# facebookresearch/GPU-DPF

Hardware: NVIDIA B200
Metric: DPFs/sec (higher is better)
Workload: dtype u32

## Files before the change

### gpu-dpf_b200/csrc/dpf_core.cuh

```cuda
#pragma once

#include <stdint.h>

#if defined(__CUDACC__)
#define DPF_HD __host__ __device__ __forceinline__
#else
#define DPF_HD inline __attribute__((always_inline))
#endif

#if defined(__CUDA_ARCH__)
#define DPF_UNROLL _Pragma("unroll")
#else
#define DPF_UNROLL
#endif

#if defined(__CUDA_ARCH__)
#define DPF_DEVICE_CODE 1
#else
#define DPF_DEVICE_CODE 0
#endif

namespace b200dpf {

enum : int { PRF_DUMMY = 0, PRF_SALSA20 = 1, PRF_CHACHA20 = 2, PRF_AES128 = 3 };

struct Seed {
    uint32_t x, y, z, w;
};

DPF_HD Seed make_seed(uint32_t x, uint32_t y, uint32_t z, uint32_t w)
{
    Seed s; s.x = x; s.y = y; s.z = z; s.w = w; return s;
}


DPF_HD uint32_t rotl(uint32_t v, int r)
{
#if DPF_DEVICE_CODE
    return __funnelshift_l(v, v, r);
#else
    return (v << r) | (v >> (32 - r));
#endif
}

#ifndef DPF_FMA_ROT_MASK
#define DPF_FMA_ROT_MASK 0
#endif
template <int R>
DPF_HD uint32_t rotl_fma(uint32_t v)
{
#if DPF_DEVICE_CODE
    uint32_t lo, hi;
    asm("{\n\t.reg .u64 t;\n\tmul.wide.u32 t, %2, %3;\n\tmov.b64 {%0,%1}, t;\n\t}"
        : "=r"(lo), "=r"(hi) : "r"(v), "n"(1u << R));
    return lo + hi;
#else
    return (v << R) | (v >> (32 - R));
#endif
}
template <int SLOT, int R>
DPF_HD uint32_t rot_sel(uint32_t v)
{
    return ((DPF_FMA_ROT_MASK >> SLOT) & 1) ? rotl_fma<R>(v) : rotl(v, R);
}

DPF_HD uint32_t prmt(uint32_t a, uint32_t b, uint32_t sel)
{
#if DPF_DEVICE_CODE
    return __byte_perm(a, b, sel);
#else
    uint64_t ab = ((uint64_t)b << 32) | a;
    uint32_t r = 0;
    for (int i = 0; i < 4; i++) {
        uint32_t n = (sel >> (4 * i)) & 7u;
        r |= (uint32_t)((ab >> (8 * n)) & 0xffu) << (8 * i);
    }
    return r;
#endif
}

DPF_HD Seed add128(const Seed &a, const Seed &b)
{
    Seed r;
#if DPF_DEVICE_CODE
    asm("add.cc.u32 %0, %4, %8;\n\t"
        "addc.cc.u32 %1, %5, %9;\n\t"
        "addc.cc.u32 %2, %6, %10;\n\t"
        "addc.u32 %3, %7, %11;"
        : "=r"(r.x), "=r"(r.y), "=r"(r.z), "=r"(r.w)
        : "r"(a.x), "r"(a.y), "r"(a.z), "r"(a.w), "r"(b.x), "r"(b.y), "r"(b.z), "r"(b.w));
#else
    uint64_t c = (uint64_t)a.x + b.x;
    r.x = (uint32_t)c; c >>= 32;
    c += (uint64_t)a.y + b.y; r.y = (uint32_t)c; c >>= 32;
    c += (uint64_t)a.z + b.z; r.z = (uint32_t)c; c >>= 32;
    c += (uint64_t)a.w + b.w; r.w = (uint32_t)c;
#endif
    return r;
}

DPF_HD Seed dummy_prf(const Seed &s, uint32_t pos)
{
    const uint64_t k = 4242ull + pos;
    Seed r;
    uint64_t t = (uint64_t)s.x * k + k;
    r.x = (uint32_t)t; t >>= 32;
    t += (uint64_t)s.y * k; r.y = (uint32_t)t; t >>= 32;
    t += (uint64_t)s.z * k; r.z = (uint32_t)t; t >>= 32;
    t += (uint64_t)s.w * k; r.w = (uint32_t)t;
    return r;
}

#define DPF_SIGMA0 0x65787061u
#define DPF_SIGMA1 0x6e642033u
#define DPF_SIGMA2 0x322d6279u
#define DPF_SIGMA3 0x7465206bu

#define DPF_SALSA_QR(a, b, c, d)      \
    do {                              \
        b ^= rot_sel<0, 7>(a + d);    \
        c ^= rot_sel<1, 9>(b + a);    \
        d ^= rot_sel<2, 13>(c + b);   \
        a ^= rot_sel<3, 18>(d + c);   \
    } while (0)

#define DPF_CHACHA_QR(a, b, c, d)     \
    do {                              \
        a += b; d = rot_sel<0, 16>(d ^ a);  \
        c += d; b = rot_sel<1, 12>(b ^ c);  \
        a += b; d = rot_sel<2, 8>(d ^ a);   \
        c += d; b = rot_sel<3, 7>(b ^ c);   \
    } while (0)

template <bool LEAF>
DPF_HD Seed salsa12(const Seed &s, uint32_t pos)
{
    const uint32_t i1 = s.w, i2 = s.z, i3 = s.y, i4 = s.x;
    uint32_t x0 = DPF_SIGMA0, x1 = i1, x2 = i2, x3 = i3, x4 = i4, x5 = DPF_SIGMA1, x6 = 0, x7 = 0,
             x8 = 0, x9 = pos, x10 = DPF_SIGMA2, x11 = 0, x12 = 0, x13 = 0, x14 = 0, x15 = DPF_SIGMA3;
DPF_UNROLL
    for (int r = 0; r < 6; r++) {
        DPF_SALSA_QR(x0, x4, x8, x12);
        DPF_SALSA_QR(x5, x9, x13, x1);
        DPF_SALSA_QR(x10, x14, x2, x6);
        DPF_SALSA_QR(x15, x3, x7, x11);
        DPF_SALSA_QR(x0, x1, x2, x3);
        DPF_SALSA_QR(x5, x6, x7, x4);
        DPF_SALSA_QR(x10, x11, x8, x9);
        DPF_SALSA_QR(x15, x12, x13, x14);
    }
    Seed o;
    o.x = x4 + i4;
    if (LEAF) { o.y = 0; o.z = 0; o.w = 0; }
    else { o.y = x3 + i3; o.z = x2 + i2; o.w = x1 + i1; }
    return o;
}

template <bool LEAF>
DPF_HD Seed chacha12(const Seed &s, uint32_t pos)
{
    const uint32_t i4 = s.w, i5 = s.z, i6 = s.y, i7 = s.x;
    uint32_t x0 = DPF_SIGMA0, x1 = DPF_SIGMA1, x2 = DPF_SIGMA2, x3 = DPF_SIGMA3, x4 = i4, x5 = i5, x6 = i6,
             x7 = i7, x8 = 0, x9 = 0, x10 = 0, x11 = 0, x12 = 0, x13 = pos, x14 = 0, x15 = 0;
DPF_UNROLL
    for (int r = 0; r < 6; r++) {
        DPF_CHACHA_QR(x0, x4, x8, x12);
        DPF_CHACHA_QR(x1, x5, x9, x13);
        DPF_CHACHA_QR(x2, x6, x10, x14);
        DPF_CHACHA_QR(x3, x7, x11, x15);
        DPF_CHACHA_QR(x0, x5, x10, x15);
        DPF_CHACHA_QR(x1, x6, x11, x12);
        DPF_CHACHA_QR(x2, x7, x8, x13);
        DPF_CHACHA_QR(x3, x4, x9, x14);
    }
    Seed o;
    o.x = x7 + i7;
    if (LEAF) { o.y = 0; o.z = 0; o.w = 0; }
    else { o.y = x6 + i6; o.z = x5 + i5; o.w = x4 + i4; }
    return o;
}

struct AesHostTables {
    const uint32_t *te0;
    template <int K, int BYTE>
    DPF_HD uint32_t te(uint32_t word) const
    {
        uint32_t v = te0[(word >> (8 * BYTE)) & 0xffu];
        return K == 0 ? v : rotl(v, 8 * K);
    }
};

template <class TA, int B0, int B1, int B2, int B3>
DPF_HD uint32_t aes_sub4(const TA &ta, uint32_t w0, uint32_t w1, uint32_t w2, uint32_t w3)
{
    const uint32_t a = ta.template te<2, B0>(w0);
    const uint32_t b = ta.template te<3, B1>(w1);
    const uint32_t c = ta.template te<0, B2>(w2);
    const uint32_t d = ta.template te<1, B3>(w3);
    const uint32_t ab = prmt(a, b, 0x0050);
    const uint32_t cd = prmt(c, d, 0x7200);
    return prmt(ab, cd, 0x7610);
}

template <class TA>
DPF_HD void aes_next_rk(const TA &ta, uint32_t &k0, uint32_t &k1, uint32_t &k2, uint32_t &k3, uint32_t rc)
{
    const uint32_t t = aes_sub4<TA, 1, 2, 3, 0>(ta, k3, k3, k3, k3);
    k0 ^= t ^ rc;
    k1 ^= k0;
    k2 ^= k1;
    k3 ^= k2;
}

template <class TA>
DPF_HD void aes_round(const TA &ta, uint32_t &s0, uint32_t &s1, uint32_t &s2, uint32_t &s3,
                      uint32_t k0, uint32_t k1, uint32_t k2, uint32_t k3)
{
    const uint32_t t0 = ta.template te<0, 0>(s0) ^ ta.template te<1, 1>(s1) ^ ta.template te<2, 2>(s2) ^ ta.template te<3, 3>(s3) ^ k0;
    const uint32_t t1 = ta.template te<0, 0>(s1) ^ ta.template te<1, 1>(s2) ^ ta.template te<2, 2>(s3) ^ ta.template te<3, 3>(s0) ^ k1;
    const uint32_t t2 = ta.template te<0, 0>(s2) ^ ta.template te<1, 1>(s3) ^ ta.template te<2, 2>(s0) ^ ta.template te<3, 3>(s1) ^ k2;
    const uint32_t t3 = ta.template te<0, 0>(s3) ^ ta.template te<1, 1>(s0) ^ ta.template te<2, 2>(s1) ^ ta.template te<3, 3>(s2) ^ k3;
    s0 = t0; s1 = t1; s2 = t2; s3 = t3;
}

template <class TA>
DPF_HD void aes_first_round(const TA &ta, uint32_t pos, uint32_t &k0, uint32_t &k1, uint32_t &k2, uint32_t &k3,
                            uint32_t &a0, uint32_t &a1, uint32_t &a2, uint32_t &a3, uint32_t &col0_te0)
{
    const uint32_t s0 = k0 ^ pos;
    const uint32_t l00 = ta.template te<0, 0>(s0), l11 = ta.template te<1, 1>(k1), l22 = ta.template te<2, 2>(k2), l33 = ta.template te<3, 3>(k3);
    const uint32_t l01 = ta.template te<0, 0>(k1), l12 = ta.template te<1, 1>(k2), l23 = ta.template te<2, 2>(k3), l30 = ta.template te<3, 3>(s0);
    const uint32_t l02 = ta.template te<0, 0>(k2), l13 = ta.template te<1, 1>(k3), l20 = ta.template te<2, 2>(s0), l31 = ta.template te<3, 3>(k1);
    const uint32_t l03 = ta.template te<0, 0>(k3), l10 = ta.template te<1, 1>(s0), l21 = ta.template te<2, 2>(k1), l32 = ta.template te<3, 3>(k2);
    const uint32_t ab = prmt(l13, l23, 0x0042);
    const uint32_t cd = prmt(l33, l03, 0x5000);
    const uint32_t t = prmt(ab, cd, 0x7610);
    k0 ^= t ^ 1u;
    k1 ^= k0;
    k2 ^= k1;
    k3 ^= k2;
    a0 = l00 ^ l11 ^ l22 ^ l33 ^ k0;
    a1 = l01 ^ l12 ^ l23 ^ l30 ^ k1;
    a2 = l02 ^ l13 ^ l20 ^ l31 ^ k2;
    a3 = l03 ^ l10 ^ l21 ^ l32 ^ k3;
    col0_te0 = l00;
}

template <bool LEAF, class TA>
DPF_HD void aes128_pair(const TA &ta, const Seed &s, Seed &c0, Seed &c1)
{
    uint32_t k0 = s.x, k1 = s.y, k2 = s.z, k3 = s.w;
    uint32_t a0, a1, a2, a3, l00;
    const uint32_t sib = ta.template te<0, 0>(k0 ^ 1u);
    aes_first_round(ta, 0u, k0, k1, k2, k3, a0, a1, a2, a3, l00);
    uint32_t b0 = a0 ^ l00 ^ sib, b1 = a1, b2 = a2, b3 = a3;
    uint32_t rc = 2;
DPF_UNROLL
    for (int r = 2; r <= 9; r++) {
        aes_next_rk(ta, k0, k1, k2, k3, rc);
        rc = (rc << 1) ^ ((rc & 0x80u) ? 0x11bu : 0u);
        aes_round(ta, a0, a1, a2, a3, k0, k1, k2, k3);
        aes_round(ta, b0, b1, b2, b3, k0, k1, k2, k3);
    }
    aes_next_rk(ta, k0, k1, k2, k3, rc);
    c0.x = aes_sub4<TA, 0, 1, 2, 3>(ta, a0, a1, a2, a3) ^ k0;
    c1.x = aes_sub4<TA, 0, 1, 2, 3>(ta, b0, b1, b2, b3) ^ k0;
    if (LEAF) {
        c0.y = c0.z = c0.w = 0;
        c1.y = c1.z = c1.w = 0;
    } else {
        c0.y = aes_sub4<TA, 0, 1, 2, 3>(ta, a1, a2, a3, a0) ^ k1;
        c0.z = aes_sub4<TA, 0, 1, 2, 3>(ta, a2, a3, a0, a1) ^ k2;
        c0.w = aes_sub4<TA, 0, 1, 2, 3>(ta, a3, a0, a1, a2) ^ k3;
        c1.y = aes_sub4<TA, 0, 1, 2, 3>(ta, b1, b2, b3, b0) ^ k1;
        c1.z = aes_sub4<TA, 0, 1, 2, 3>(ta, b2, b3, b0, b1) ^ k2;
        c1.w = aes_sub4<TA, 0, 1, 2, 3>(ta, b3, b0, b1, b2) ^ k3;
    }
}

template <class TA>
DPF_HD Seed aes128_one(const TA &ta, const Seed &s, uint32_t pos)
{
    uint32_t k0 = s.x, k1 = s.y, k2 = s.z, k3 = s.w;
    uint32_t a0, a1, a2, a3, l00;
    aes_first_round(ta, pos, k0, k1, k2, k3, a0, a1, a2, a3, l00);
    uint32_t rc = 2;
DPF_UNROLL
    for (int r = 2; r <= 9; r++) {
        aes_next_rk(ta, k0, k1, k2, k3, rc);
        rc = (rc << 1) ^ ((rc & 0x80u) ? 0x11bu : 0u);
        aes_round(ta, a0, a1, a2, a3, k0, k1, k2, k3);
    }
    aes_next_rk(ta, k0, k1, k2, k3, rc);
    Seed c;
    c.x = aes_sub4<TA, 0, 1, 2, 3>(ta, a0, a1, a2, a3) ^ k0;
    c.y = aes_sub4<TA, 0, 1, 2, 3>(ta, a1, a2, a3, a0) ^ k1;
    c.z = aes_sub4<TA, 0, 1, 2, 3>(ta, a2, a3, a0, a1) ^ k2;
    c.w = aes_sub4<TA, 0, 1, 2, 3>(ta, a3, a0, a1, a2) ^ k3;
    return c;
}


template <int PRF, bool LEAF, class TA>
DPF_HD void expand_pair(const TA &ta, const Seed &parent, Seed &c0, Seed &c1)
{
    if (PRF == PRF_DUMMY) {
        c0 = dummy_prf(parent, 0);
        c1 = dummy_prf(parent, 1);
    } else if (PRF == PRF_SALSA20) {
        c0 = salsa12<LEAF>(parent, 0);
        c1 = salsa12<LEAF>(parent, 1);
    } else if (PRF == PRF_CHACHA20) {
        c0 = chacha12<LEAF>(parent, 0);
        c1 = chacha12<LEAF>(parent, 1);
    } else {
        aes128_pair<LEAF>(ta, parent, c0, c1);
    }
}

template <int PRF, class TA>
DPF_HD Seed expand_one(const TA &ta, const Seed &parent, uint32_t pos)
{
    if (PRF == PRF_DUMMY) return dummy_prf(parent, pos);
    if (PRF == PRF_SALSA20) return salsa12<false>(parent, pos);
    if (PRF == PRF_CHACHA20) return chacha12<false>(parent, pos);
    return aes128_one(ta, parent, pos);
}


template <int PRF, class Env>
DPF_HD Seed walk_down(Env &env, Seed seed, int first_level, int steps, uint32_t q)
{
    for (int k = 0; k < steps; k++) {
        const uint32_t bit = (q >> (steps - 1 - k)) & 1u;
        const int level = first_level - k;
        const uint32_t bank = seed.x & 1u;
        seed = add128(expand_one<PRF>(env.ta, seed, bit), env.cw(level, bank, bit));
    }
    return seed;
}

DPF_HD int ctz32(uint32_t v)
{
#if DPF_DEVICE_CODE
    return __ffs((int)v) - 1;
#else
    return __builtin_ctz(v);
#endif
}

template <int PRF, bool FULL, class Env>
DPF_HD void eval_subtree(Env &env, Seed seed, int s, int level_base)
{
    int h = s;
    const uint32_t npairs = 1u << (s - 1);
    for (uint32_t i = 0; i < npairs; i++) {
        while (h > 1) {
            Seed c0, c1;
            expand_pair<PRF, false>(env.ta, seed, c0, c1);
            const uint32_t bank = seed.x & 1u;
            const int level = level_base + h - 1;
            c1 = add128(c1, env.cw(level, bank, 1));
            env.push(h - 1, c1);
            seed = add128(c0, env.cw(level, bank, 0));
            h--;
        }
        Seed l0, l1;
        const uint32_t bank = seed.x & 1u;
        if (FULL) {
            expand_pair<PRF, false>(env.ta, seed, l0, l1);
            env.node_pair(2 * i, add128(l0, env.cw(level_base, bank, 0)), add128(l1, env.cw(level_base, bank, 1)));
        } else {
            env.leaf_prefetch(2 * i);
            expand_pair<PRF, true>(env.ta, seed, l0, l1);
            env.leaf_pair(2 * i, l0.x + env.cw_lo(bank, 0), l1.x + env.cw_lo(bank, 1));
        }
        h = ctz32(i + 1) + 1;
        if (h < s) seed = env.pop(h);
    }
}

}
```

### gpu-dpf_b200/csrc/dpf_kernels.cu

```cuda
#include "dpf_kernels.cuh"

#include <algorithm>
#include <atomic>

#include "dpf_core.cuh"

namespace b200dpf {

namespace {

__constant__ uint32_t c_te0[256];

struct AesSmemTables {
    uint32_t lanebase;

    template <int K, int BYTE>
    __device__ __forceinline__ uint32_t te(uint32_t word) const
    {
        const uint32_t addr = __byte_perm(word, lanebase, 0x7604u | (BYTE << 4));
        uint32_t v;
        asm("ld.shared.u32 %0, [%1+%2];" : "=r"(v) : "r"(addr), "n"((K & 1) * 128 + (K >> 1) * 65536));
        return v;
    }
};

struct NoTables {
    template <int K, int BYTE>
    __device__ __forceinline__ uint32_t te(uint32_t) const { return 0; }
};

template <int PRF> struct TablePolicy { typedef NoTables type; };
template <> struct TablePolicy<PRF_AES128> { typedef AesSmemTables type; };

namespace tma {

__device__ __forceinline__ void mbar_init(uint32_t bar, uint32_t count)
{
    asm volatile("mbarrier.init.shared::cta.b64 [%0], %1;" ::"r"(bar), "r"(count));
}
__device__ __forceinline__ void mbar_expect_tx(uint32_t bar, uint32_t bytes)
{
    asm volatile("mbarrier.arrive.expect_tx.shared::cta.b64 _, [%0], %1;" ::"r"(bar), "r"(bytes) : "memory");
}
__device__ __forceinline__ void mbar_arrive(uint32_t bar)
{
    asm volatile("mbarrier.arrive.shared::cta.b64 _, [%0];" ::"r"(bar) : "memory");
}
__device__ __forceinline__ void mbar_wait(uint32_t bar, uint32_t parity)
{
    uint32_t done = 0;
    for (uint32_t spin = 0; !done; spin++) {
        asm volatile("{\n\t.reg .pred p;\n\tmbarrier.try_wait.parity.shared::cta.b64 p, [%1], %2;\n\tselp.u32 %0, 1, 0, p;\n\t}"
                     : "=r"(done) : "r"(bar), "r"(parity) : "memory");
        if (spin > (1u << 28)) __trap();
    }
}
__device__ __forceinline__ void bulk_g2s(uint32_t dst, const void *src, uint32_t bytes, uint32_t bar)
{
    asm volatile("cp.async.bulk.shared::cluster.global.mbarrier::complete_tx::bytes [%0], [%1], %2, [%3];"
                 ::"r"(dst), "l"(src), "r"(bytes), "r"(bar) : "memory");
}

}

template <int PRF, int NV, int THREADS, int MODE>
struct DevEnv {
    typename TablePolicy<PRF>::type ta;
    const uint4 *cw_lane;
    const uint32_t *cwlo_lane;
    uint4 *stack_lo, *stack_hi;
    int stack_split;
    const uint4 *rows;
    uint32_t row_stride_v;
    uint32_t acc[4 * NV];
    uint4 ra[4], rb[4];
    uint32_t *leaf_out;
    uint4 *front_out;
    uint32_t kpw;
    uint32_t *share_row;
    uint32_t pos_base;
    int depth;
    bool key_valid;

    __device__ __forceinline__ Seed cw(int level, uint32_t bank, uint32_t bit) const
    {
        const uint4 v = cw_lane[((level * 2 + (int)bank) * 2 + (int)bit) * 32];
        return make_seed(v.x, v.y, v.z, v.w);
    }
    __device__ __forceinline__ uint32_t cw_lo(uint32_t bank, uint32_t bit) const
    {
        return cwlo_lane[(bank * 2 + bit) * 32];
    }
    __device__ __forceinline__ uint4 *slot(int h) const
    {
        const int l = h - 1;
        return (l < stack_split ? stack_lo : stack_hi) + l * THREADS;
    }
    __device__ __forceinline__ void push(int h, const Seed &s) const
    {
        *slot(h) = make_uint4(s.x, s.y, s.z, s.w);
    }
    __device__ __forceinline__ Seed pop(int h) const
    {
        const uint4 v = *slot(h);
        return make_seed(v.x, v.y, v.z, v.w);
    }
    static constexpr bool MAC = (MODE == MODE_FUSED || MODE == MODE_GROUPED || MODE == MODE_FUSED_TMA);
    static constexpr bool STAGED = (MODE == MODE_FUSED_TMA);
    const uint4 *tile;
    uint32_t tile_bar;
    uint32_t tile_phase;
    bool tile_pending;

    __device__ __forceinline__ void leaf_prefetch(uint32_t local_pos)
    {
        if (STAGED) {
            if (tile_pending) {
                tma::mbar_wait(tile_bar, tile_phase);
                tile_phase ^= 1u;
                tile_pending = false;
            }
            const uint4 *r = tile + (size_t)local_pos * 4;
#pragma unroll
            for (int j = 0; j < 4; j++) ra[j] = r[j];
#pragma unroll
            for (int j = 0; j < 4; j++) rb[j] = r[4 + j];
        } else if (MAC) {
            const uint4 *r = rows + (size_t)local_pos * row_stride_v;
#pragma unroll
            for (int j = 0; j < 4; j++) ra[j] = __ldg(r + j);
#pragma unroll
            for (int j = 0; j < 4; j++) rb[j] = __ldg(r + row_stride_v + j);
        }
    }
    __device__ __forceinline__ void leaf_pair(uint32_t local_pos, uint32_t v0, uint32_t v1)
    {
        if (MAC) {
            if (leaf_out != nullptr) {
                leaf_out[(size_t)local_pos * 32] = v0;
                leaf_out[(size_t)(local_pos + 1) * 32] = v1;
            }
            const uint4 *r = rows + (size_t)local_pos * row_stride_v;
#pragma unroll
            for (int c = 0; c < NV / 4; c++) {
                uint4 na[4], nb[4];
                if (c + 1 < NV / 4) {
#pragma unroll
                    for (int j = 0; j < 4; j++) na[j] = __ldg(r + 4 * (c + 1) + j);
#pragma unroll
                    for (int j = 0; j < 4; j++) nb[j] = __ldg(r + row_stride_v + 4 * (c + 1) + j);
                }
#pragma unroll
                for (int j = 0; j < 4; j++) {
                    acc[16 * c + 4 * j + 0] += v0 * ra[j].x + v1 * rb[j].x;
                    acc[16 * c + 4 * j + 1] += v0 * ra[j].y + v1 * rb[j].y;
                    acc[16 * c + 4 * j + 2] += v0 * ra[j].z + v1 * rb[j].z;
                    acc[16 * c + 4 * j + 3] += v0 * ra[j].w + v1 * rb[j].w;
                }
                if (c + 1 < NV / 4) {
#pragma unroll
                    for (int j = 0; j < 4; j++) { ra[j] = na[j]; rb[j] = nb[j]; }
                }
            }
        } else if (MODE == MODE_EXPAND && key_valid) {
            const uint32_t p = pos_base + local_pos;
            share_row[__brev(p) >> (32 - depth)] = v0;
            share_row[__brev(p + 1) >> (32 - depth)] = v1;
        }
    }
    __device__ __forceinline__ void node_pair(uint32_t local_pos, const Seed &c0, const Seed &c1)
    {
        front_out[(size_t)local_pos * kpw] = make_uint4(c0.x, c0.y, c0.z, c0.w);
        front_out[(size_t)(local_pos + 1) * kpw] = make_uint4(c1.x, c1.y, c1.z, c1.w);
    }
};

template <int PRF, int NV> struct KernelShape { enum { THREADS = (NV <= 8 ? 256 : 384), MIN_BLOCKS = (NV <= 8 ? 2 : 1) }; };
#ifndef DPF_AES_THREADS
#define DPF_AES_THREADS 384
#endif
template <int NV> struct KernelShape<PRF_AES128, NV> { enum { THREADS = (NV <= 8 ? DPF_AES_THREADS : 256), MIN_BLOCKS = 1 }; };

extern __shared__ __align__(16) unsigned char g_dyn_smem[];

__device__ __forceinline__ void grid_barrier(uint32_t *bar, uint32_t target)
{
    __syncthreads();
    if (threadIdx.x == 0) {
        __threadfence();
        atomicAdd(bar, 1u);
        for (uint32_t spin = 0;; spin++) {
            uint32_t v;
            asm volatile("ld.acquire.gpu.global.u32 %0, [%1];" : "=r"(v) : "l"(bar) : "memory");
            if ((int32_t)(v - target) >= 0) break;
            if (spin > (1u << 25)) __trap();
            __nanosleep(40);
        }
        __threadfence();
    }
    __syncthreads();
}

__device__ __forceinline__ unsigned long long global_ns()
{
    unsigned long long t;
    asm volatile("mov.u64 %0, %globaltimer;" : "=l"(t));
    return t;
}

template <int PRF, int NV, int THREADS, int MODE>
__device__ __forceinline__ void run_phase(const EvalParams &p, const PhaseParams &ph,
                                          const typename TablePolicy<PRF>::type &ta, uint32_t quota = 0xffffffffu)
{
    const int tid = threadIdx.x;
    const int lane = tid & 31;

    uint4 *cw_s = reinterpret_cast<uint4 *>(g_dyn_smem + p.off_cw);
    uint32_t *cwlo_s = reinterpret_cast<uint32_t *>(g_dyn_smem + p.off_cwlo);
    uint4 *root_s = reinterpret_cast<uint4 *>(g_dyn_smem + p.off_root);
    volatile int *flag_s = reinterpret_cast<volatile int *>(g_dyn_smem + p.off_flag);

    const int kpw = 1 << p.kpw_log2;
    const int spw_log2 = 5 - p.kpw_log2;
    const int kslot = lane & (kpw - 1);
    const uint32_t sslot = (uint32_t)lane >> p.kpw_log2;
    const uint32_t ntickets = ph.nsub >> spw_log2;

    DevEnv<PRF, NV, THREADS, MODE> env;
    env.ta = ta;
    env.cw_lane = cw_s + kslot;
    env.cwlo_lane = cwlo_s + kslot;
    env.kpw = (uint32_t)kpw;
    env.stack_lo = reinterpret_cast<uint4 *>(g_dyn_smem + p.off_stack_lo) + tid;
    env.stack_hi = reinterpret_cast<uint4 *>(g_dyn_smem + p.off_stack_hi) + tid - ph.stack_split * THREADS;
    env.stack_split = ph.stack_split;
    env.row_stride_v = p.row_stride_v;
    env.depth = p.depth;
    if constexpr (MODE == MODE_FUSED_TMA) {
        const int w = tid >> 5;
        env.tile = reinterpret_cast<const uint4 *>(g_dyn_smem + p.off_tile + ((size_t)w << (ph.s + 6)));
        env.tile_bar = (uint32_t)__cvta_generic_to_shared(g_dyn_smem + p.off_tile_bar + 8 * w);
        env.tile_phase = 0;
        env.tile_pending = false;
        if (lane == 0) {
            tma::mbar_init(env.tile_bar, 1);
            asm volatile("fence.mbarrier_init.release.cluster;" ::: "memory");
        }
        __syncwarp();
    }

    constexpr bool GROUPED = (MODE == MODE_GROUPED);
    uint32_t taken = 0;
    for (int j = 0; j < p.key_groups; j++) {
        const int kg = (int)((blockIdx.x + (unsigned)j) % (unsigned)p.key_groups);

        int g_depth = p.depth, g_s = ph.s, g_walk_first = ph.walk_first_level, g_walk_steps = ph.walk_steps;
        int g_key_first = kg * kpw, g_key_last = p.nkeys - 1;
        uint32_t g_tickets = ntickets;
        const uint4 *g_table = p.table;
        if (GROUPED) {
            const GroupDesc g = p.groups[kg];
            g_depth = g.depth;
            g_s = g.s;
            g_walk_first = g.depth - 1;
            g_walk_steps = g.depth - g.s;
            g_key_first = (int)g.key_first;
            g_key_last = (int)(g.key_first + g.nkeys) - 1;
            g_tickets = g.nsub;
            g_table = p.table + g.table_off_v;
        }

        if (quota != 0xffffffffu && __syncthreads_and(taken >= quota)) break;
        if (tid == 0) *flag_s = (*reinterpret_cast<volatile uint32_t *>(ph.counters + kg) < g_tickets) ? 1 : 0;
        __syncthreads();
        const bool has_work = (*flag_s != 0);
        if (has_work) {
            const int per_key = g_depth * 4;
            for (int i = tid; i < per_key * kpw; i += THREADS) {
                const int k = i / per_key;
                const int e = i - k * per_key;
                const int bank = e / (g_depth * 2);
                const int lb = e - bank * (g_depth * 2);
                int key = g_key_first + k;
                if (key > g_key_last) key = g_key_last;
                const int level = lb >> 1, bit = lb & 1;
                const uint32_t slot = p.key_compact ? 2u + 4u * (uint32_t)level + 2u * (uint32_t)bank + (uint32_t)bit
                                                    : (bank ? 65u : 1u) + (uint32_t)lb;
                const uint4 v = __ldg(p.keys + (size_t)key * p.key_stride_v + slot);
                cw_s[((level * 2 + bank) * 2 + bit) * 32 + k] = v;
                if (level == 0) cwlo_s[(bank * 2 + bit) * 32 + k] = v.x;
            }
            if (tid < kpw) {
                int key = g_key_first + tid;
                if (key > g_key_last) key = g_key_last;
                root_s[tid] = __ldg(p.keys + (size_t)key * p.key_stride_v + p.key_root_v);
            }
        }
        __syncthreads();
        if (!has_work) continue;

        const int key = g_key_first + kslot;
        env.key_valid = key <= g_key_last;
        if (MODE == MODE_FUSED || MODE == MODE_FUSED_TMA || GROUPED) {
#pragma unroll
            for (int e = 0; e < 4 * NV; e++) env.acc[e] = 0;
        } else if (MODE == MODE_EXPAND) {
            env.share_row = p.shares + (size_t)(env.key_valid ? key : 0) * p.n;
        }
        const uint4 rv = root_s[kslot];
        const Seed root = make_seed(rv.x, rv.y, rv.z, rv.w);

        const uint32_t grid_warps = gridDim.x * (uint32_t)(THREADS / 32);
        const bool chunked = quota == 0xffffffffu;
        const bool ahead = g_s <= 4;
        uint32_t chunk = 1;
        if (chunked) chunk = min(8u, max(1u, g_tickets / (8u * grid_warps)));
        uint32_t t_raw = 0;
        bool draw = taken < quota;
        if (draw && lane == 0) t_raw = atomicAdd(ph.counters + kg, chunk);
        while (draw) {
            const uint32_t t0 = __shfl_sync(0xffffffffu, t_raw, 0);
            if (t0 >= g_tickets) break;
            const uint32_t t1 = min(t0 + chunk, g_tickets);
            taken += t1 - t0;
            draw = taken < quota;
            if (chunked) chunk = min(8u, max(1u, (g_tickets - t1) / (8u * grid_warps)));
            if (ahead && draw && lane == 0) t_raw = atomicAdd(ph.counters + kg, chunk);
          for (uint32_t t = t0; t < t1; t++) {
            const uint32_t q = (t << spw_log2) + sslot;
            Seed start = root;
            if (ph.frontier_in != nullptr) {
                const uint4 fv = __ldcg(ph.frontier_in + ((size_t)kg * p.nfront + (q >> ph.front_shift)) * kpw + kslot);
                start = make_seed(fv.x, fv.y, fv.z, fv.w);
            }
            const Seed r = walk_down<PRF>(env, start, g_walk_first, g_walk_steps, ph.sub_first + q);
            if (MODE == MODE_FRONTIER) {
                env.front_out = p.frontier_out + ((size_t)kg * p.nfront + ((size_t)q << g_s)) * kpw + kslot;
                eval_subtree<PRF, true>(env, r, g_s, ph.level_base);
            } else {
                env.rows = g_table + ((size_t)q << g_s) * p.row_stride_v + p.col_off_v;
                if constexpr (MODE == MODE_FUSED_TMA) {
                    __syncwarp();
                    if (lane == 0) {
                        asm volatile("fence.proxy.async.shared::cta;" ::: "memory");
                        const uint32_t bytes = 64u << g_s;
                        tma::mbar_expect_tx(env.tile_bar, bytes);
                        tma::bulk_g2s((uint32_t)__cvta_generic_to_shared(const_cast<uint4 *>(env.tile)), env.rows, bytes, env.tile_bar);
                    }
                    env.tile_pending = true;
                }
                env.pos_base = (ph.sub_first + q) << g_s;
                env.leaf_out = (!GROUPED && p.leaf_cache) ? p.leaf_cache + ((size_t)kg * p.n_local + ((size_t)q << g_s)) * 32 + lane
                                                          : nullptr;
                eval_subtree<PRF, false>(env, r, g_s, 0);
            }
          }
            if (!ahead && draw && lane == 0) t_raw = atomicAdd(ph.counters + kg, chunk);
        }

        if (MODE == MODE_FUSED || MODE == MODE_FUSED_TMA || GROUPED) {
            for (int off = kpw; off < 32; off <<= 1) {
#pragma unroll
                for (int e = 0; e < 4 * NV; e++) env.acc[e] += __shfl_xor_sync(0xffffffffu, env.acc[e], off);
            }
            if (env.key_valid && sslot == 0) {
                uint32_t *o = p.out + (size_t)key * p.out_stride + p.col_off;
#pragma unroll
                for (int e = 0; e < 4 * NV; e++)
                    if ((uint32_t)e < p.ncols) atomicAdd(o + e, env.acc[e]);
            }
        }
        __syncthreads();
    }
}

template <int PRF, int NV, int MODE>
__global__ void __launch_bounds__((KernelShape<PRF, NV>::THREADS), (KernelShape<PRF, NV>::MIN_BLOCKS))
dpf_eval_kernel(const __grid_constant__ EvalParams p)
{
    constexpr int THREADS = KernelShape<PRF, NV>::THREADS;
    const int tid = threadIdx.x;
    unsigned long long *stamp = (p.timing != nullptr && tid == 0) ? p.timing + (size_t)blockIdx.x * 8 : nullptr;
    if (stamp) stamp[0] = global_ns();

    typename TablePolicy<PRF>::type ta;
    if constexpr (PRF == PRF_AES128) {
        const uint32_t tab = (uint32_t)__cvta_generic_to_shared(g_dyn_smem + p.off_tab);
        if ((tab & 0xffffu) != 0) __trap();
        for (int i = tid; i < 256 * 32; i += THREADS) {
            const uint32_t v = c_te0[i >> 5];
            unsigned char *e = g_dyn_smem + p.off_tab + (i >> 5) * 256 + (i & 31) * 4;
            *reinterpret_cast<uint32_t *>(e) = v;
            *reinterpret_cast<uint32_t *>(e + 128) = __funnelshift_l(v, v, 8);
            *reinterpret_cast<uint32_t *>(e + 65536) = __funnelshift_l(v, v, 16);
            *reinterpret_cast<uint32_t *>(e + 65536 + 128) = __funnelshift_l(v, v, 24);
        }
        ta.lanebase = tab + (tid & 31) * 4;
    }

    if constexpr (MODE != MODE_FRONTIER) {
        if (p.fuse_top) {
            const uint64_t gtid = (uint64_t)blockIdx.x * THREADS + tid, gthreads = (uint64_t)gridDim.x * THREADS;
            for (uint64_t i = gtid; i < p.zero_a_words; i += gthreads) p.zero_a[i] = 0u;
            for (uint64_t i = gtid; i < p.zero_b_words; i += gthreads) p.zero_b[i] = 0u;
            if (stamp) stamp[1] = global_ns();
            if (p.top.nsub != 0) {
                constexpr uint32_t NW = THREADS / 32;
                const uint32_t w = (uint32_t)tid >> 5;
                uint32_t bq = p.top_block_quota;
                const uint32_t kgs = (uint32_t)p.key_groups;
                if (bq != 0x7fffffffu && gridDim.x >= kgs) {
                    const uint32_t nb = gridDim.x / kgs + ((blockIdx.x % kgs) < (gridDim.x % kgs) ? 1u : 0u);
                    const uint32_t tickets = p.top.nsub >> (5 - p.kpw_log2);
                    bq = (tickets + nb - 1) / nb;
                }
                run_phase<PRF, 4, THREADS, MODE_FRONTIER>(p, p.top, ta, bq / NW + (w < bq % NW ? 1u : 0u));
                run_phase<PRF, 4, THREADS, MODE_FRONTIER>(p, p.top, ta);
            }
            if (stamp) stamp[2] = global_ns();
            grid_barrier(p.grid_bar, p.grid_bar_target);
            if (stamp) stamp[3] = global_ns();
            if (blockIdx.x == 0)
                for (uint32_t i = tid; i < p.rearm_words; i += THREADS) p.rearm[i] = 0u;
        }
    }
    run_phase<PRF, NV, THREADS, MODE>(p, p.main, ta);
    if (stamp) stamp[4] = global_ns();
}

template <int NV>
__global__ void __launch_bounds__(256, 2) dpf_mac_kernel(const __grid_constant__ MacParams p)
{
    const int lane = threadIdx.x & 31;
    const uint64_t warp_global = ((uint64_t)blockIdx.x * blockDim.x + threadIdx.x) >> 5;
    const uint64_t warps_total = ((uint64_t)gridDim.x * blockDim.x) >> 5;
    const uint64_t items = (uint64_t)p.key_groups * p.ranges_per_group;
    const uint64_t len = (p.n_local + p.ranges_per_group - 1) / p.ranges_per_group;
    for (uint64_t w = warp_global; w < items; w += warps_total) {
        const uint32_t kg = (uint32_t)(w / p.ranges_per_group);
        const uint32_t r = (uint32_t)(w - (uint64_t)kg * p.ranges_per_group);
        const uint64_t begin = (uint64_t)r * len;
        const uint64_t end = begin + len < p.n_local ? begin + len : p.n_local;
        uint32_t acc[4 * NV];
#pragma unroll
        for (int e = 0; e < 4 * NV; e++) acc[e] = 0;
        const uint32_t *leaf = p.leaf_cache + ((size_t)kg * p.n_local + begin) * 32 + lane;
        const uint4 *row = p.table + begin * p.row_stride_v + p.col_off_v;
        uint64_t pos = begin;
        for (; pos + 4 <= end; pos += 4) {
            uint32_t v[4];
#pragma unroll
            for (int u = 0; u < 4; u++) v[u] = __ldg(leaf + 32 * u);
#pragma unroll
            for (int j = 0; j < NV; j++) {
                uint4 t[4];
#pragma unroll
                for (int u = 0; u < 4; u++) t[u] = __ldg(row + (size_t)u * p.row_stride_v + j);
#pragma unroll
                for (int u = 0; u < 4; u++) {
                    acc[4 * j + 0] += v[u] * t[u].x;
                    acc[4 * j + 1] += v[u] * t[u].y;
                    acc[4 * j + 2] += v[u] * t[u].z;
                    acc[4 * j + 3] += v[u] * t[u].w;
                }
            }
            leaf += 128;
            row += (size_t)4 * p.row_stride_v;
        }
        for (; pos < end; pos++) {
            const uint32_t v = __ldg(leaf);
#pragma unroll
            for (int j = 0; j < NV; j++) {
                const uint4 t = __ldg(row + j);
                acc[4 * j + 0] += v * t.x;
                acc[4 * j + 1] += v * t.y;
                acc[4 * j + 2] += v * t.z;
                acc[4 * j + 3] += v * t.w;
            }
            leaf += 32;
            row += p.row_stride_v;
        }
        const int key = (int)kg * 32 + lane;
        if (key < p.nkeys) {
            uint32_t *o = p.out + (size_t)key * p.out_stride + p.col_off;
#pragma unroll
            for (int e = 0; e < 4 * NV; e++)
                if ((uint32_t)e >= p.col_skip && (uint32_t)e < p.ncols) atomicAdd(o + e, acc[e]);
        }
    }
}


template <int NV>
struct MacTmaShape {
    enum { P = 32, STAGES = 3, GROUPS = 8, ROW_BYTES = NV * 16, LEAF_TILE = P * 128,
           STAGE_BYTES = GROUPS * LEAF_TILE + P * ROW_BYTES, SMEM = STAGES * STAGE_BYTES + 64,
           THREADS = (GROUPS + 1) * 32 };
};

template <int NV>
__global__ void __launch_bounds__(MacTmaShape<NV>::THREADS, 1) dpf_mac_tma_kernel(const __grid_constant__ MacParams p)
{
    typedef MacTmaShape<NV> S;
    const int lane = threadIdx.x & 31;
    const int warp = threadIdx.x >> 5;
    const uint32_t smem0 = (uint32_t)__cvta_generic_to_shared(g_dyn_smem);
    const uint32_t bars = smem0 + S::STAGES * S::STAGE_BYTES;
    if (threadIdx.x == 0) {
        for (int i = 0; i < S::STAGES; i++) {
            tma::mbar_init(bars + 8 * i, 1);
            tma::mbar_init(bars + 8 * (S::STAGES + i), S::GROUPS);
        }
        asm volatile("fence.mbarrier_init.release.cluster;" ::: "memory");
    }
    __syncthreads();

    const uint32_t kg_blocks = ((uint32_t)p.key_groups + S::GROUPS - 1) / S::GROUPS;
    const uint64_t items = (uint64_t)kg_blocks * p.ranges_per_group;
    const uint64_t len = (p.n_local + p.ranges_per_group - 1) / p.ranges_per_group;
    uint32_t seq = 0;

    for (uint64_t it = blockIdx.x; it < items; it += gridDim.x) {
        const uint32_t kgb = (uint32_t)(it / p.ranges_per_group);
        const uint32_t r = (uint32_t)(it - (uint64_t)kgb * p.ranges_per_group);
        const uint64_t begin = (uint64_t)r * len;
        const uint64_t end = begin + len < p.n_local ? begin + len : p.n_local;
        const uint32_t kg0 = kgb * S::GROUPS;
        const uint32_t ngroups = min((uint32_t)S::GROUPS, (uint32_t)p.key_groups - kg0);

        if (warp == S::GROUPS) {
            for (uint64_t pos = begin; pos < end; pos += S::P, seq++) {
                const uint32_t stage = seq % S::STAGES, phase = (seq / S::STAGES) & 1u;
                const uint32_t cnt = (uint32_t)min((uint64_t)S::P, end - pos);
                const uint32_t sbase = smem0 + stage * S::STAGE_BYTES;
                const uint32_t full = bars + 8 * stage, empty = bars + 8 * (S::STAGES + stage);
                tma::mbar_wait(empty, phase ^ 1u);
                if (lane == 0) tma::mbar_expect_tx(full, cnt * (128u * ngroups + S::ROW_BYTES));
                __syncwarp();
                if ((uint32_t)lane < ngroups)
                    tma::bulk_g2s(sbase + lane * S::LEAF_TILE,
                                  p.leaf_cache + ((size_t)(kg0 + lane) * p.n_local + pos) * 32, cnt * 128u, full);
                for (uint32_t i = lane; i < cnt; i += 32)
                    tma::bulk_g2s(sbase + S::GROUPS * S::LEAF_TILE + i * S::ROW_BYTES,
                                  p.table + (pos + i) * p.row_stride_v + p.col_off_v, S::ROW_BYTES, full);
            }
        } else {
            const bool active = (uint32_t)warp < ngroups;
            uint32_t acc[4 * NV];
#pragma unroll
            for (int e = 0; e < 4 * NV; e++) acc[e] = 0;
            for (uint64_t pos = begin; pos < end; pos += S::P, seq++) {
                const uint32_t stage = seq % S::STAGES, phase = (seq / S::STAGES) & 1u;
                const uint32_t cnt = (uint32_t)min((uint64_t)S::P, end - pos);
                const unsigned char *sbase = g_dyn_smem + stage * S::STAGE_BYTES;
                tma::mbar_wait(bars + 8 * stage, phase);
                if (active) {
                    const uint32_t *leaf = reinterpret_cast<const uint32_t *>(sbase + warp * S::LEAF_TILE) + lane;
                    const uint4 *rows = reinterpret_cast<const uint4 *>(sbase + S::GROUPS * S::LEAF_TILE);
#pragma unroll 2
                    for (uint32_t i = 0; i < cnt; i++) {
                        const uint32_t v = leaf[i * 32];
#pragma unroll
                        for (int j = 0; j < NV; j++) {
                            const uint4 t = rows[i * NV + j];
                            acc[4 * j + 0] += v * t.x;
                            acc[4 * j + 1] += v * t.y;
                            acc[4 * j + 2] += v * t.z;
                            acc[4 * j + 3] += v * t.w;
                        }
                    }
                }
                __syncwarp();
                if (lane == 0) tma::mbar_arrive(bars + 8 * (S::STAGES + stage));
            }
            const int key = (int)(kg0 + warp) * 32 + lane;
            if (active && key < p.nkeys) {
                uint32_t *o = p.out + (size_t)key * p.out_stride + p.col_off;
#pragma unroll
                for (int e = 0; e < 4 * NV; e++)
                    if ((uint32_t)e >= p.col_skip && (uint32_t)e < p.ncols) atomicAdd(o + e, acc[e]);
            }
        }
    }
}

__global__ void __launch_bounds__(256) sum_partials_kernel(uint32_t *__restrict__ dst, const PeerParts parts, size_t words)
{
    const size_t tid = (size_t)blockIdx.x * blockDim.x + threadIdx.x, nthr = (size_t)gridDim.x * blockDim.x;
    if ((words & 3u) == 0) {
        uint4 *d4 = reinterpret_cast<uint4 *>(dst);
        for (size_t i = tid; i < words / 4; i += nthr) {
            uint4 a = d4[i];
            for (int k = 0; k < parts.n; k++) {
                const uint4 b = __ldcg(reinterpret_cast<const uint4 *>(parts.p[k]) + i);
                a.x += b.x; a.y += b.y; a.z += b.z; a.w += b.w;
            }
            d4[i] = a;
        }
    } else {
        for (size_t i = tid; i < words; i += nthr) {
            uint32_t a = dst[i];
            for (int k = 0; k < parts.n; k++) a += __ldcg(parts.p[k] + i);
            dst[i] = a;
        }
    }
}

__global__ void probe_smem_kernel(uint32_t *out)
{
    if (threadIdx.x == 0) *out = (uint32_t)__cvta_generic_to_shared(g_dyn_smem);
}

__global__ void permute_table_kernel(const int32_t *__restrict__ stage, int32_t *__restrict__ table,
                                     uint64_t rows, int bits, int cols, int stride)
{
    const uint64_t total = rows * (uint64_t)cols;
    for (uint64_t i = (uint64_t)blockIdx.x * blockDim.x + threadIdx.x; i < total;
         i += (uint64_t)gridDim.x * blockDim.x) {
        const uint64_t q = i / (uint64_t)cols;
        const int c = (int)(i - q * (uint64_t)cols);
        const uint64_t src = bits ? (uint64_t)(__brev((uint32_t)q) >> (32 - bits)) : 0;
        table[q * (uint64_t)stride + c] = stage[src * (uint64_t)cols + c];
    }
}

template <int PRF, int NV, int MODE>
cudaError_t launch_one(const EvalParams &p, int grid, size_t smem, cudaStream_t stream)
{
    auto kern = dpf_eval_kernel<PRF, NV, MODE>;
    static std::atomic<int> configured[64];
    int dev = 0;
    cudaError_t e = cudaGetDevice(&dev);
    if (e != cudaSuccess) return e;
    if (dev < 0 || dev >= 64 || configured[dev].load(std::memory_order_acquire) != (int)smem + 1) {
        e = cudaFuncSetAttribute(kern, cudaFuncAttributeMaxDynamicSharedMemorySize, (int)smem);
        if (e != cudaSuccess) return e;
        e = cudaFuncSetAttribute(kern, cudaFuncAttributePreferredSharedMemoryCarveout, cudaSharedmemCarveoutMaxShared);
        if (e != cudaSuccess) return e;
        if (dev >= 0 && dev < 64) configured[dev].store((int)smem + 1, std::memory_order_release);
    }
    if (p.fuse_top) {
        void *args[] = {const_cast<EvalParams *>(&p)};
        return cudaLaunchCooperativeKernel(reinterpret_cast<const void *>(kern), dim3((unsigned)grid),
                                           dim3((unsigned)(KernelShape<PRF, NV>::THREADS)), args, smem, stream);
    }
    kern<<<grid, (KernelShape<PRF, NV>::THREADS), smem, stream>>>(p);
    return cudaGetLastError();
}

template <int PRF, int NV, int MODE>
cudaError_t max_smem_one(int *bytes)
{
    cudaFuncAttributes a;
    cudaError_t e = cudaFuncGetAttributes(&a, dpf_eval_kernel<PRF, NV, MODE>);
    if (e != cudaSuccess) return e;
    int dev = 0, optin = 0;
    if ((e = cudaGetDevice(&dev)) != cudaSuccess) return e;
    if ((e = cudaDeviceGetAttribute(&optin, cudaDevAttrMaxSharedMemoryPerBlockOptin, dev)) != cudaSuccess) return e;
    *bytes = optin - (int)a.sharedSizeBytes;
    return cudaSuccess;
}

template <int PRF>
cudaError_t launch_prf(int nv, int mode, const EvalParams &p, int grid, size_t smem, cudaStream_t stream)
{
    if (mode == MODE_EXPAND) return launch_one<PRF, 4, MODE_EXPAND>(p, grid, smem, stream);
    if (mode == MODE_FRONTIER) return launch_one<PRF, 4, MODE_FRONTIER>(p, grid, smem, stream);
    if (mode == MODE_GROUPED) return launch_one<PRF, 4, MODE_GROUPED>(p, grid, smem, stream);
    if (mode == MODE_FUSED_TMA) {
        if constexpr (PRF == PRF_AES128) return cudaErrorInvalidValue;
        else return launch_one<PRF, 4, MODE_FUSED_TMA>(p, grid, smem, stream);
    }
    if (nv == 4) return launch_one<PRF, 4, MODE_FUSED>(p, grid, smem, stream);
    if (nv == 8) return launch_one<PRF, 8, MODE_FUSED>(p, grid, smem, stream);
    if (nv == 16) return launch_one<PRF, 16, MODE_FUSED>(p, grid, smem, stream);
    return cudaErrorInvalidValue;
}

template <int PRF>
cudaError_t max_smem_prf(int nv, int mode, int *bytes)
{
    if (mode == MODE_EXPAND) return max_smem_one<PRF, 4, MODE_EXPAND>(bytes);
    if (mode == MODE_FRONTIER) return max_smem_one<PRF, 4, MODE_FRONTIER>(bytes);
    if (mode == MODE_GROUPED) return max_smem_one<PRF, 4, MODE_GROUPED>(bytes);
    if (mode == MODE_FUSED_TMA) {
        if constexpr (PRF == PRF_AES128) return cudaErrorInvalidValue;
        else return max_smem_one<PRF, 4, MODE_FUSED_TMA>(bytes);
    }
    if (nv == 4) return max_smem_one<PRF, 4, MODE_FUSED>(bytes);
    if (nv == 8) return max_smem_one<PRF, 8, MODE_FUSED>(bytes);
    if (nv == 16) return max_smem_one<PRF, 16, MODE_FUSED>(bytes);
    return cudaErrorInvalidValue;
}

}

int eval_threads(int prf, int nv)
{
    if (prf == PRF_AES128) return nv <= 8 ? DPF_AES_THREADS : 256;
    return nv <= 8 ? 256 : 384;
}

int eval_min_blocks(int prf, int nv)
{
    if (prf == PRF_AES128) return 1;
    return nv <= 8 ? 2 : 1;
}

cudaError_t probe_dynamic_smem_base(uint32_t *base, cudaStream_t stream)
{
    uint32_t *d = nullptr;
    cudaError_t e = cudaMalloc(&d, sizeof(uint32_t));
    if (e != cudaSuccess) return e;
    probe_smem_kernel<<<1, 32, 16, stream>>>(d);
    e = cudaGetLastError();
    if (e == cudaSuccess) e = cudaMemcpyAsync(base, d, sizeof(uint32_t), cudaMemcpyDeviceToHost, stream);
    if (e == cudaSuccess) e = cudaStreamSynchronize(stream);
    cudaFree(d);
    return e;
}

cudaError_t upload_aes_table(const uint32_t *te0_256)
{
    return cudaMemcpyToSymbol(c_te0, te0_256, 256 * sizeof(uint32_t));
}

cudaError_t launch_eval(int prf, int nv, int mode, const EvalParams &p, int grid, size_t smem, cudaStream_t stream)
{
    switch (prf) {
    case PRF_DUMMY: return launch_prf<PRF_DUMMY>(nv, mode, p, grid, smem, stream);
    case PRF_SALSA20: return launch_prf<PRF_SALSA20>(nv, mode, p, grid, smem, stream);
    case PRF_CHACHA20: return launch_prf<PRF_CHACHA20>(nv, mode, p, grid, smem, stream);
    case PRF_AES128: return launch_prf<PRF_AES128>(nv, mode, p, grid, smem, stream);
    default: return cudaErrorInvalidValue;
    }
}

cudaError_t eval_max_smem(int prf, int nv, int mode, int *bytes)
{
    switch (prf) {
    case PRF_DUMMY: return max_smem_prf<PRF_DUMMY>(nv, mode, bytes);
    case PRF_SALSA20: return max_smem_prf<PRF_SALSA20>(nv, mode, bytes);
    case PRF_CHACHA20: return max_smem_prf<PRF_CHACHA20>(nv, mode, bytes);
    case PRF_AES128: return max_smem_prf<PRF_AES128>(nv, mode, bytes);
    default: return cudaErrorInvalidValue;
    }
}

cudaError_t launch_mac_tma(const MacParams &p, int grid, cudaStream_t stream)
{
    typedef MacTmaShape<16> S;
    auto kern = dpf_mac_tma_kernel<16>;
    static std::atomic<int> configured[64];
    int dev = 0;
    cudaError_t e = cudaGetDevice(&dev);
    if (e != cudaSuccess) return e;
    if (dev < 0 || dev >= 64 || !configured[dev].load(std::memory_order_acquire)) {
        e = cudaFuncSetAttribute(kern, cudaFuncAttributeMaxDynamicSharedMemorySize, (int)S::SMEM);
        if (e != cudaSuccess) return e;
        if (dev >= 0 && dev < 64) configured[dev].store(1, std::memory_order_release);
    }
    kern<<<grid, (int)S::THREADS, (int)S::SMEM, stream>>>(p);
    return cudaGetLastError();
}

cudaError_t launch_mac(int nv, const MacParams &p, int grid, cudaStream_t stream)
{
    if (nv == 4) dpf_mac_kernel<4><<<grid, 256, 0, stream>>>(p);
    else if (nv == 8) dpf_mac_kernel<8><<<grid, 256, 0, stream>>>(p);
    else if (nv == 16) dpf_mac_kernel<16><<<grid, 256, 0, stream>>>(p);
    else return cudaErrorInvalidValue;
    return cudaGetLastError();
}

cudaError_t launch_sum_partials(uint32_t *dst, const PeerParts &parts, size_t words, cudaStream_t stream)
{
    if (parts.n <= 0 || words == 0) return cudaSuccess;
    int grid = (int)std::min<size_t>((words / 4 + 255) / 256 + 1, 148 * 4);
    sum_partials_kernel<<<grid, 256, 0, stream>>>(dst, parts, words);
    return cudaGetLastError();
}

cudaError_t launch_permute_table(const int32_t *stage, int32_t *table, uint64_t rows, int bits,
                                 int cols, int stride, cudaStream_t stream)
{
    const uint64_t total = rows * (uint64_t)cols;
    int grid = (int)((total + 255) / 256);
    if (grid > 148 * 16) grid = 148 * 16;
    if (grid < 1) grid = 1;
    permute_table_kernel<<<grid, 256, 0, stream>>>(stage, table, rows, bits, cols, stride);
    return cudaGetLastError();
}

}
```

Baseline: 25210.

## Split MAC row columns across quad lanes and keep last sibling in registers

```diff
diff --git a/gpu-dpf_b200/csrc/dpf_core.cuh b/gpu-dpf_b200/csrc/dpf_core.cuh
--- a/gpu-dpf_b200/csrc/dpf_core.cuh
+++ b/gpu-dpf_b200/csrc/dpf_core.cuh
@@ -353,6 +353,8 @@
 DPF_HD void eval_subtree(Env &env, Seed seed, int s, int level_base)
 {
     int h = s;
+    constexpr bool REG_SIBLING = (PRF == PRF_AES128);
+    Seed right1 = seed;
     const uint32_t npairs = 1u << (s - 1);
     for (uint32_t i = 0; i < npairs; i++) {
         while (h > 1) {
@@ -361,7 +363,8 @@
             const uint32_t bank = seed.x & 1u;
             const int level = level_base + h - 1;
             c1 = add128(c1, env.cw(level, bank, 1));
-            env.push(h - 1, c1);
+            if (REG_SIBLING && h == 2) right1 = c1;
+            else env.push(h - 1, c1);
             seed = add128(c0, env.cw(level, bank, 0));
             h--;
         }
@@ -376,8 +379,9 @@
             env.leaf_pair(2 * i, l0.x + env.cw_lo(bank, 0), l1.x + env.cw_lo(bank, 1));
         }
         h = ctz32(i + 1) + 1;
-        if (h < s) seed = env.pop(h);
-    }
-}
-
-}
+        if (REG_SIBLING && h == 1 && s > 1) seed = right1;
+        else if (h < s) seed = env.pop(h);
+    }
+}
+
+}
diff --git a/gpu-dpf_b200/csrc/dpf_kernels.cu b/gpu-dpf_b200/csrc/dpf_kernels.cu
--- a/gpu-dpf_b200/csrc/dpf_kernels.cu
+++ b/gpu-dpf_b200/csrc/dpf_kernels.cu
@@ -63,8 +63,9 @@
 
 }
 
-template <int PRF, int NV, int THREADS, int MODE>
+template <int PRF, int NV, int THREADS, int MODE, bool QUAD>
 struct DevEnv {
+    static constexpr int ROW_V = QUAD ? NV / 4 : 4;
     typename TablePolicy<PRF>::type ta;
     const uint4 *cw_lane;
     const uint32_t *cwlo_lane;
@@ -72,8 +73,9 @@
     int stack_split;
     const uint4 *rows;
     uint32_t row_stride_v;
+    uint32_t qlane;
     uint32_t acc[4 * NV];
-    uint4 ra[4], rb[4];
+    uint4 ra[ROW_V], rb[ROW_V];
     uint32_t *leaf_out;
     uint4 *front_out;
     uint32_t kpw;
@@ -114,52 +116,86 @@
 
     __device__ __forceinline__ void leaf_prefetch(uint32_t local_pos)
     {
-        if (STAGED) {
+        if constexpr (STAGED) {
             if (tile_pending) {
                 tma::mbar_wait(tile_bar, tile_phase);
                 tile_phase ^= 1u;
                 tile_pending = false;
             }
             const uint4 *r = tile + (size_t)local_pos * 4;
-#pragma unroll
-            for (int j = 0; j < 4; j++) ra[j] = r[j];
-#pragma unroll
-            for (int j = 0; j < 4; j++) rb[j] = r[4 + j];
-        } else if (MAC) {
-            const uint4 *r = rows + (size_t)local_pos * row_stride_v;
-#pragma unroll
-            for (int j = 0; j < 4; j++) ra[j] = __ldg(r + j);
-#pragma unroll
-            for (int j = 0; j < 4; j++) rb[j] = __ldg(r + row_stride_v + j);
+            if constexpr (QUAD) {
+                ra[0] = r[qlane];
+                rb[0] = r[4 + qlane];
+            } else {
+#pragma unroll
+                for (int j = 0; j < 4; j++) ra[j] = r[j];
+#pragma unroll
+                for (int j = 0; j < 4; j++) rb[j] = r[4 + j];
+            }
+        } else if constexpr (MAC) {
+            if constexpr (QUAD) {
+                const uint4 *r = rows + (size_t)local_pos * row_stride_v + qlane;
+#pragma unroll
+                for (int c = 0; c < ROW_V; c++) ra[c] = __ldg(r + 4 * c);
+#pragma unroll
+                for (int c = 0; c < ROW_V; c++) rb[c] = __ldg(r + row_stride_v + 4 * c);
+            } else {
+                const uint4 *r = rows + (size_t)local_pos * row_stride_v;
+#pragma unroll
+                for (int j = 0; j < 4; j++) ra[j] = __ldg(r + j);
+#pragma unroll
+                for (int j = 0; j < 4; j++) rb[j] = __ldg(r + row_stride_v + j);
+            }
         }
     }
     __device__ __forceinline__ void leaf_pair(uint32_t local_pos, uint32_t v0, uint32_t v1)
     {
-        if (MAC) {
+        if constexpr (MAC) {
             if (leaf_out != nullptr) {
                 leaf_out[(size_t)local_pos * 32] = v0;
                 leaf_out[(size_t)(local_pos + 1) * 32] = v1;
             }
-            const uint4 *r = rows + (size_t)local_pos * row_stride_v;
-#pragma unroll
-            for (int c = 0; c < NV / 4; c++) {
-                uint4 na[4], nb[4];
-                if (c + 1 < NV / 4) {
-#pragma unroll
-                    for (int j = 0; j < 4; j++) na[j] = __ldg(r + 4 * (c + 1) + j);
-#pragma unroll
-                    for (int j = 0; j < 4; j++) nb[j] = __ldg(r + row_stride_v + 4 * (c + 1) + j);
+            if constexpr (QUAD) {
+                uint32_t w0[4], w1[4];
+                w0[0] = v0;
+                w1[0] = v1;
+#pragma unroll
+                for (int m = 1; m < 4; m++) {
+                    w0[m] = __shfl_xor_sync(0xffffffffu, v0, m);
+                    w1[m] = __shfl_xor_sync(0xffffffffu, v1, m);
                 }
 #pragma unroll
-                for (int j = 0; j < 4; j++) {
-                    acc[16 * c + 4 * j + 0] += v0 * ra[j].x + v1 * rb[j].x;
-                    acc[16 * c + 4 * j + 1] += v0 * ra[j].y + v1 * rb[j].y;
-                    acc[16 * c + 4 * j + 2] += v0 * ra[j].z + v1 * rb[j].z;
-                    acc[16 * c + 4 * j + 3] += v0 * ra[j].w + v1 * rb[j].w;
+                for (int c = 0; c < ROW_V; c++) {
+#pragma unroll
+                    for (int m = 0; m < 4; m++) {
+                        acc[16 * c + 4 * m + 0] += w0[m] * ra[c].x + w1[m] * rb[c].x;
+                        acc[16 * c + 4 * m + 1] += w0[m] * ra[c].y + w1[m] * rb[c].y;
+                        acc[16 * c + 4 * m + 2] += w0[m] * ra[c].z + w1[m] * rb[c].z;
+                        acc[16 * c + 4 * m + 3] += w0[m] * ra[c].w + w1[m] * rb[c].w;
+                    }
                 }
-                if (c + 1 < NV / 4) {
-#pragma unroll
-                    for (int j = 0; j < 4; j++) { ra[j] = na[j]; rb[j] = nb[j]; }
+            } else {
+                const uint4 *r = rows + (size_t)local_pos * row_stride_v;
+#pragma unroll
+                for (int c = 0; c < NV / 4; c++) {
+                    uint4 na[4], nb[4];
+                    if (c + 1 < NV / 4) {
+#pragma unroll
+                        for (int j = 0; j < 4; j++) na[j] = __ldg(r + 4 * (c + 1) + j);
+#pragma unroll
+                        for (int j = 0; j < 4; j++) nb[j] = __ldg(r + row_stride_v + 4 * (c + 1) + j);
+                    }
+#pragma unroll
+                    for (int j = 0; j < 4; j++) {
+                        acc[16 * c + 4 * j + 0] += v0 * ra[j].x + v1 * rb[j].x;
+                        acc[16 * c + 4 * j + 1] += v0 * ra[j].y + v1 * rb[j].y;
+                        acc[16 * c + 4 * j + 2] += v0 * ra[j].z + v1 * rb[j].z;
+                        acc[16 * c + 4 * j + 3] += v0 * ra[j].w + v1 * rb[j].w;
+                    }
+                    if (c + 1 < NV / 4) {
+#pragma unroll
+                        for (int j = 0; j < 4; j++) { ra[j] = na[j]; rb[j] = nb[j]; }
+                    }
                 }
             }
         } else if (MODE == MODE_EXPAND && key_valid) {
@@ -208,7 +244,7 @@
     return t;
 }
 
-template <int PRF, int NV, int THREADS, int MODE>
+template <int PRF, int NV, int THREADS, int MODE, bool QUAD = false>
 __device__ __forceinline__ void run_phase(const EvalParams &p, const PhaseParams &ph,
                                           const typename TablePolicy<PRF>::type &ta, uint32_t quota = 0xffffffffu)
 {
@@ -226,8 +262,9 @@
     const uint32_t sslot = (uint32_t)lane >> p.kpw_log2;
     const uint32_t ntickets = ph.nsub >> spw_log2;
 
-    DevEnv<PRF, NV, THREADS, MODE> env;
+    DevEnv<PRF, NV, THREADS, MODE, QUAD> env;
     env.ta = ta;
+    env.qlane = (uint32_t)lane & 3u;
     env.cw_lane = cw_s + kslot;
     env.cwlo_lane = cwlo_s + kslot;
     env.kpw = (uint32_t)kpw;
@@ -363,7 +400,21 @@
 #pragma unroll
                 for (int e = 0; e < 4 * NV; e++) env.acc[e] += __shfl_xor_sync(0xffffffffu, env.acc[e], off);
             }
-            if (env.key_valid && sslot == 0) {
+            if (QUAD && sslot == 0) {
+#pragma unroll
+                for (int m = 0; m < 4; m++) {
+                    const int key_m = g_key_first + (kslot ^ m);
+                    if (key_m > g_key_last) continue;
+                    uint32_t *o = p.out + (size_t)key_m * p.out_stride + p.col_off;
+#pragma unroll
+                    for (int c = 0; c < NV / 4; c++)
+#pragma unroll
+                        for (int e = 0; e < 4; e++) {
+                            const uint32_t col = 4u * (4u * c + env.qlane) + e;
+                            if (col < p.ncols) atomicAdd(o + col, env.acc[16 * c + 4 * m + e]);
+                        }
+                }
+            } else if (!QUAD && env.key_valid && sslot == 0) {
                 uint32_t *o = p.out + (size_t)key * p.out_stride + p.col_off;
 #pragma unroll
                 for (int e = 0; e < 4 * NV; e++)
@@ -424,7 +475,13 @@
                 for (uint32_t i = tid; i < p.rearm_words; i += THREADS) p.rearm[i] = 0u;
         }
     }
-    run_phase<PRF, NV, THREADS, MODE>(p, p.main, ta);
+    constexpr bool QUAD_MAC = PRF != PRF_CHACHA20;
+    if constexpr (QUAD_MAC && (MODE == MODE_FUSED || MODE == MODE_GROUPED || MODE == MODE_FUSED_TMA)) {
+        if (p.kpw_log2 >= 2) run_phase<PRF, NV, THREADS, MODE, true>(p, p.main, ta);
+        else run_phase<PRF, NV, THREADS, MODE, false>(p, p.main, ta);
+    } else {
+        run_phase<PRF, NV, THREADS, MODE>(p, p.main, ta);
+    }
     if (stamp) stamp[4] = global_ns();
 }
 
```

Measured after the change: 26040 (median of 6 runs). +3.3%, better.
